# mborhi/CoMA-UNet

Measured on AMD Instinct MI355X. Metric: volumes/sec (train fwd+bwd) at 128^3 bf16, higher is better.
Workload: dtype bf16; 1 GPU; CoMA-UNet train step (fwd + RoiMSE/RnC loss + bwd + all-reduce + AdamW), 128^3 volumes, batch 2/GPU, 6-dim covariates (BASELINE configs[3]); global_batch=2, parallelism=dp1, launch=hipGraph replay of the whole step

## Files before the change

### coma_unet_amd/csrc/conv_mfma.hip

```cpp
#include "conv_mfma.h"
#include <type_traits>

template <typename T> struct elem;
template <> struct elem<bf16_t> { static constexpr int EPB = 8; };
template <> struct elem<float> { static constexpr int EPB = 4; };

__device__ __forceinline__ f32x16_t mma_piece(const uint4& a, const uint4& b, f32x16_t acc, bf16_t) {
  return __builtin_amdgcn_mfma_f32_32x32x16_bf16(*reinterpret_cast<const bf16x8_t*>(&a), *reinterpret_cast<const bf16x8_t*>(&b), acc, 0, 0, 0);
}
__device__ __forceinline__ f32x16_t mma_piece(const uint4& a, const uint4& b, f32x16_t acc, float) {
  acc = __builtin_amdgcn_mfma_f32_32x32x2f32(__uint_as_float(a.x), __uint_as_float(b.x), acc, 0, 0, 0);
  acc = __builtin_amdgcn_mfma_f32_32x32x2f32(__uint_as_float(a.y), __uint_as_float(b.y), acc, 0, 0, 0);
  acc = __builtin_amdgcn_mfma_f32_32x32x2f32(__uint_as_float(a.z), __uint_as_float(b.z), acc, 0, 0, 0);
  acc = __builtin_amdgcn_mfma_f32_32x32x2f32(__uint_as_float(a.w), __uint_as_float(b.w), acc, 0, 0, 0);
  return acc;
}

struct GatherP {
  const void* x; int ldx; long sbx; int Di, Hi, Wi, C;
  void* y; int ldy; long sby; int Do, Ho, Wo, N;
  const void* w; long wsb;
  const float* bias; int bsb;
  int k, stride, flip;
  int Mz, My, Mx;
// ... 2731 lines not shown
  extern __shared__ __attribute__((aligned(16))) char smem[];
  float* Hl = reinterpret_cast<float*>(smem);
  float* Dl = Hl + HV * CP;
  const int tid = threadIdx.x, lane = tid & 63;
  const int wid = __builtin_amdgcn_readfirstlane(tid >> 6);
  const int b = blockIdx.z;
  const int lv = lane & 15, lg = lane >> 4;
  const float* xb = p.x + (long)b * p.sbx;
  const float* db = p.dy + (long)b * p.sbn;
  const __amdgpu_buffer_rsrc_t rs_x = __builtin_amdgcn_make_buffer_rsrc(const_cast<float*>(xb), 0, p.xbytes, 0x00020000);
  const __amdgpu_buffer_rsrc_t rs_d = __builtin_amdgcn_make_buffer_rsrc(const_cast<float*>(db), 0, p.dbytes, 0x00020000);
  constexpr unsigned OOB = 0x7fff0000u;

  int s_z[NIT], s_y[NIT], s_x[NIT];
  unsigned s_boff[NIT];
#pragma unroll
  for (int it = 0; it < NIT; ++it) {
    if (it < HIT) {
      const int piece = tid + 256 * it;
      const int row = piece / PCH, ch = piece % PCH;
      const int hx = row % HX, hy = (row / HX) % HY, hz = row / (HX * HY);
      s_z[it] = piece < HP ? hz - 1 : (1 << 20); s_y[it] = hy - 1; s_x[it] = hx - 1;
      s_boff[it] = (unsigned)(ch * 16);
    } else {
      const int piece = tid + 256 * (it - HIT);
      const int row = piece / DCH, ch = piece % DCH;
      s_z[it] = row >> 7; s_y[it] = (row >> 5) & 3; s_x[it] = row & 31;
      s_boff[it] = (unsigned)(ch * 16);
    }
  }
  const int xval = p.C - 4 * (tid % PCH), dval = p.N - 4 * (tid % DCH);
  const uint4 xmask = make_uint4(xval > 0 ? ~0u : 0u, xval > 1 ? ~0u : 0u, xval > 2 ? ~0u : 0u, xval > 3 ? ~0u : 0u);
  const uint4 dmask = make_uint4(dval > 0 ? ~0u : 0u, dval > 1 ? ~0u : 0u, dval > 2 ? ~0u : 0u, dval > 3 ? ~0u : 0u);
  uint4 sreg[NIT];
  auto issue = [&](int it, int z0, int y0, int x0, const __amdgpu_buffer_rsrc_t& rx, const __amdgpu_buffer_rsrc_t& rd) __attribute__((always_inline)) {
    const int gz = z0 + s_z[it], gy = y0 + s_y[it], gx = x0 + s_x[it];
    const bool ok = (unsigned)gz < (unsigned)p.D && (unsigned)gy < (unsigned)p.H && (unsigned)gx < (unsigned)p.W;
    const int ld = it < HIT ? p.ldx : p.ldn;
    const unsigned off = (unsigned)(((gz * p.H + gy) * p.W + gx) * ld) * 4u + s_boff[it];
    const auto v = __builtin_amdgcn_raw_buffer_load_b128(it < HIT ? rx : rd, ok ? off : OOB, 0, 0);
    sreg[it] = make_uint4(v[0], v[1], v[2], v[3]);
  };
  auto store_tile = [&]() __attribute__((always_inline)) {
#pragma unroll
    for (int it = 0; it < NIT; ++it) {
      uint4 v = sreg[it];
      if (it < HIT) {
        if (tid + 256 * it < HP) {
          v.x &= xmask.x; v.y &= xmask.y; v.z &= xmask.z; v.w &= xmask.w;
          reinterpret_cast<uint4*>(Hl)[tid + 256 * it] = v;
        }
      } else {
        v.x &= dmask.x; v.y &= dmask.y; v.z &= dmask.z; v.w &= dmask.w;
        reinterpret_cast<uint4*>(Dl)[tid + 256 * (it - HIT)] = v;
      }
    }
  };

  const int gz = wid >> 1, gy0 = 2 * (wid & 1);
  const int dbase = ((gz * 4 + gy0) * 32 + lg) * ND + lv;
  const int sub = lv / CP, cc = lv % CP;
  const int xbase = ((gz * HY + gy0) * HX + lg) * CP + cc;
  int toff[NM];
#pragma unroll
  for (int m = 0; m < NM; ++m) {
    const int t = TPM == 1 ? m : (m * TPM + sub < 27 ? m * TPM + sub : 0);
    toff[m] = (((t / 9) * HY + (t / 3) % 3) * HX + t % 3) * CP;
  }
  f32x4_t acc[NM][NB];
#pragma unroll
  for (int m = 0; m < NM; ++m)
#pragma unroll
    for (int nb = 0; nb < NB; ++nb) acc[m][nb] = (f32x4_t){0.f, 0.f, 0.f, 0.f};

  const int id_begin = xcd_remap(blockIdx.x, gridDim.x) * p.ids_per_block;
  int id_end = id_begin + p.ids_per_block;
  if (id_end > p.ids_total) id_end = p.ids_total;
  int id = id_begin, tix = 0, tiy = 0, tiz = 0;
  while (id < id_end && !tile_coords(id, p.ntx, p.nty, p.ntz, tix, tiy, tiz)) ++id;
  if (id < id_end) {
#pragma unroll
    for (int it = 0; it < NIT; ++it) issue(it, tiz * TZ, tiy * TY, tix * TX, rs_x, rs_d);
  }
  while (id < id_end) {
    int nid = id + 1, ntix = 0, ntiy = 0, ntiz = 0;
    while (nid < id_end && !tile_coords(nid, p.ntx, p.nty, p.ntz, ntix, ntiy, ntiz)) ++nid;
    const bool has_next = nid < id_end;
    const __amdgpu_buffer_rsrc_t rn_x = __builtin_amdgcn_make_buffer_rsrc(const_cast<float*>(xb), 0, has_next ? p.xbytes : 0, 0x00020000);
    const __amdgpu_buffer_rsrc_t rn_d = __builtin_amdgcn_make_buffer_rsrc(const_cast<float*>(db), 0, has_next ? p.dbytes : 0, 0x00020000);
    __syncthreads();
    store_tile();
    __syncthreads();
    float af[2][NB], bf[2][NM];
    auto rd = [&](int s_, int buf) __attribute__((always_inline)) {
      const int so_d = ((s_ >> 3) * 32 + 4 * (s_ & 7)) * ND, so_x = ((s_ >> 3) * HX + 4 * (s_ & 7)) * CP;
#pragma unroll
      for (int nb = 0; nb < NB; ++nb) af[buf][nb] = Dl[dbase + so_d + nb * 16];
#pragma unroll
      for (int m = 0; m < NM; ++m) bf[buf][m] = Hl[xbase + so_x + toff[m]];
    };
    rd(0, 0);
#pragma unroll
    for (int s_ = 0; s_ < 16; ++s_) {
      if (s_ + 1 < 16) rd(s_ + 1, (s_ + 1) & 1);
      if (s_ < NIT) issue(s_, ntiz * TZ, ntiy * TY, ntix * TX, rn_x, rn_d);
      if (s_ + 16 < NIT) issue(s_ + 16, ntiz * TZ, ntiy * TY, ntix * TX, rn_x, rn_d);
      __builtin_amdgcn_sched_barrier(0);
#pragma unroll
      for (int m = 0; m < NM; ++m)
#pragma unroll
        for (int nb = 0; nb < NB; ++nb)
          acc[m][nb] = __builtin_amdgcn_mfma_f32_16x16x4f32(af[s_ & 1][nb], bf[s_ & 1][m], acc[m][nb], 0, 0, 0);
      __builtin_amdgcn_sched_barrier(0);
    }
    id = nid; tix = ntix; tiy = ntiy; tiz = ntiz;
  }
  __syncthreads();
  float* red = reinterpret_cast<float*>(smem);
  for (int i = tid; i < NM * NB * 256; i += 256) red[i] = 0.f;
  __syncthreads();
#pragma unroll
  for (int m = 0; m < NM; ++m)
#pragma unroll
    for (int nb = 0; nb < NB; ++nb)
#pragma unroll
      for (int j = 0; j < 4; ++j) atomicAdd(&red[((m * NB + nb) * 16 + 4 * lg + j) * 16 + lv], acc[m][nb][j]);
  __syncthreads();
  float* wout = p.dwk + (long)b * p.wsb + (long)(blockIdx.x % (unsigned)p.nrep) * p.rep_stride;
  for (int i = tid; i < NM * NB * 256; i += 256) {
    const int col = i & 15, row = (i >> 4) & 15, nb = (i >> 8) % NB, m = i / (256 * NB);
    const int tap = m * TPM + col / CP, c = col % CP, n = nb * 16 + row;
    if (tap < 27 && n < p.N && c < p.C) atomicAdd(wout + ((long)tap * p.N + n) * p.C + c, red[i]);
  }
}

struct Thin16WP {
  const bf16_t* x; int ldx; long sbx; int D, H, W, C;
  const bf16_t* dy; int ldn; long sbn; int N;
  unsigned xbytes, dbytes;
  int ntx, nty, ntz, ids_total, ids_per_block;
  float* dwk; long wsb;
  int nrep; long rep_stride;
};

template <int CP, int NB>
__global__ __launch_bounds__(256, 2) void conv_thin16_wgrad_k(Thin16WP p) {
  constexpr int TX = 32, TY = 4, TZ = 2, HX = TX + 2, HY = TY + 2, HZ = TZ + 2, HV = HX * HY * HZ, TM = TX * TY * TZ;
  constexpr int TPM = 16 / CP, NM = (27 + TPM - 1) / TPM;
  constexpr int ND = NB * 16;
  constexpr int PX = CP * 2, PD = ND * 2;
  constexpr int PCH = CP / 8, DCH = ND / 8;
  constexpr int HP = HV * PCH, DP = TM * DCH, HIT = (HP + 255) / 256, DIT = DP / 256, NIT = HIT + DIT;
  constexpr int RING = 8;
  extern __shared__ __attribute__((aligned(16))) char smem[];
  char* Hl = smem;
  char* Dl = smem + (HV + 2) * PX;
  const int tid = threadIdx.x, lane = tid & 63;
  const int wid = __builtin_amdgcn_readfirstlane(tid >> 6);
  const int b = blockIdx.z;
  const int lv = lane & 15, lg = lane >> 4;
  const bf16_t* xb = p.x + (long)b * p.sbx;
  const bf16_t* db = p.dy + (long)b * p.sbn;
  const __amdgpu_buffer_rsrc_t rs_x = __builtin_amdgcn_make_buffer_rsrc(const_cast<bf16_t*>(xb), 0, p.xbytes, 0x00020000);
  const __amdgpu_buffer_rsrc_t rs_d = __builtin_amdgcn_make_buffer_rsrc(const_cast<bf16_t*>(db), 0, p.dbytes, 0x00020000);
  constexpr unsigned OOB = 0x7fff0000u;

  int s_z[NIT], s_y[NIT], s_x[NIT];
#pragma unroll
  for (int it = 0; it < NIT; ++it) {
    if (it < HIT) {
      const int piece = tid + 256 * it;
      const int row = piece / PCH;
      const int hx = row % HX, hy = (row / HX) % HY, hz = row / (HX * HY);
      s_z[it] = piece < HP ? hz - 1 : (1 << 20); s_y[it] = hy - 1; s_x[it] = hx - 1;
    } else {
      const int row = (tid + 256 * (it - HIT)) / DCH;
      s_z[it] = row >> 7; s_y[it] = (row >> 5) & 3; s_x[it] = row & 31;
    }
  }
  const unsigned xoffb = (unsigned)((tid % PCH) * 16), doffb = (unsigned)((tid % DCH) * 16);
  const uint4 xmask = mask8(p.C - 8 * (tid % PCH)), dmask = mask8(p.N - 8 * (tid % DCH));
  uint4 sreg[NIT];
  auto issue = [&](int it, int z0, int y0, int x0, const __amdgpu_buffer_rsrc_t& rx, const __amdgpu_buffer_rsrc_t& rd) __attribute__((always_inline)) {
    const int gz = z0 + s_z[it], gy = y0 + s_y[it], gx = x0 + s_x[it];
    const bool ok = (unsigned)gz < (unsigned)p.D && (unsigned)gy < (unsigned)p.H && (unsigned)gx < (unsigned)p.W;
    const unsigned off = (unsigned)(((gz * p.H + gy) * p.W + gx) * (it < HIT ? p.ldx : p.ldn)) * 2u + (it < HIT ? xoffb : doffb);
    const auto v = __builtin_amdgcn_raw_buffer_load_b128(it < HIT ? rx : rd, ok ? off : OOB, 0, 0);
    sreg[it] = make_uint4(v[0], v[1], v[2], v[3]);
  };
  auto store_tile = [&]() __attribute__((always_inline)) {
#pragma unroll
    for (int it = 0; it < NIT; ++it) {
      uint4 v = sreg[it];
      if (it < HIT) {
        if (tid + 256 * it < HP) {
          v.x &= xmask.x; v.y &= xmask.y; v.z &= xmask.z; v.w &= xmask.w;
          reinterpret_cast<uint4*>(Hl)[tid + 256 * it] = v;
        }
      } else {
        v.x &= dmask.x; v.y &= dmask.y; v.z &= dmask.z; v.w &= dmask.w;
        reinterpret_cast<uint4*>(Dl)[tid + 256 * (it - HIT)] = v;
      }
    }
  };

  const int gz = wid >> 1, gy0 = 2 * (wid & 1);
  const int q4 = lv >> 2, p4 = lv & 3;
  const int vx = 4 * lg + q4;
  const int d_addr = ((gz * 4 + gy0) * 32 + vx) * PD + 8 * p4;
  const int sub = (4 * p4) / CP, cin = (4 * p4) % CP;
  const int x_addr = ((gz * HY + gy0) * HX + vx) * PX + cin * 2;
  int toff[NM];
#pragma unroll
  for (int m = 0; m < NM; ++m) {
    const int t = TPM == 1 ? m : (m * TPM + sub < 27 ? m * TPM + sub : 0);
    toff[m] = (((t / 9) * HY + (t / 3) % 3) * HX + t % 3) * PX;
  }
  f32x4_t acc[NM][NB];
#pragma unroll
  for (int m = 0; m < NM; ++m)
#pragma unroll
    for (int nb = 0; nb < NB; ++nb) acc[m][nb] = (f32x4_t){0.f, 0.f, 0.f, 0.f};

  const int id_begin = xcd_remap(blockIdx.x, gridDim.x) * p.ids_per_block;
  int id_end = id_begin + p.ids_per_block;
  if (id_end > p.ids_total) id_end = p.ids_total;
  int id = id_begin, tix = 0, tiy = 0, tiz = 0;
  while (id < id_end && !tile_coords(id, p.ntx, p.nty, p.ntz, tix, tiy, tiz)) ++id;
  if (id < id_end) {
#pragma unroll
    for (int it = 0; it < NIT; ++it) issue(it, tiz * TZ, tiy * TY, tix * TX, rs_x, rs_d);
  }
  while (id < id_end) {
    int nid = id + 1, ntix = 0, ntiy = 0, ntiz = 0;
    while (nid < id_end && !tile_coords(nid, p.ntx, p.nty, p.ntz, ntix, ntiy, ntiz)) ++nid;
    const bool has_next = nid < id_end;
    const __amdgpu_buffer_rsrc_t rn_x = __builtin_amdgcn_make_buffer_rsrc(const_cast<bf16_t*>(xb), 0, has_next ? p.xbytes : 0, 0x00020000);
    const __amdgpu_buffer_rsrc_t rn_d = __builtin_amdgcn_make_buffer_rsrc(const_cast<bf16_t*>(db), 0, has_next ? p.dbytes : 0, 0x00020000);
    __syncthreads();
    store_tile();
    __syncthreads();
    constexpr int NPAIR = 2 * NM;
    bf16x8_t bring[RING];
    auto rdb = [&](int pi) __attribute__((always_inline)) -> bf16x8_t {
      const int s_ = pi / NM, m = pi % NM;
      const char* src = Hl + x_addr + s_ * HX * PX + toff[m];
      const s4_t lo = __builtin_amdgcn_ds_read_tr16_b64_v4i16((lds_s4_t*)(src));
      const s4_t hi = __builtin_amdgcn_ds_read_tr16_b64_v4i16((lds_s4_t*)(src + 16 * PX));
      return (bf16x8_t){lo[0], lo[1], lo[2], lo[3], hi[0], hi[1], hi[2], hi[3]};
    };
    auto rda = [&](int s_, int nb) __attribute__((always_inline)) -> bf16x8_t {
      const char* src = Dl + d_addr + s_ * 32 * PD + nb * 32;
      const s4_t lo = __builtin_amdgcn_ds_read_tr16_b64_v4i16((lds_s4_t*)(src));
      const s4_t hi = __builtin_amdgcn_ds_read_tr16_b64_v4i16((lds_s4_t*)(src + 16 * PD));
      return (bf16x8_t){lo[0], lo[1], lo[2], lo[3], hi[0], hi[1], hi[2], hi[3]};
    };
    bf16x8_t afr[2][NB];
#pragma unroll
    for (int s_ = 0; s_ < 2; ++s_)
#pragma unroll
      for (int nb = 0; nb < NB; ++nb) afr[s_][nb] = rda(s_, nb);
#pragma unroll
    for (int pi = 0; pi < RING && pi < NPAIR; ++pi) bring[pi] = rdb(pi);
#pragma unroll
    for (int pi = 0; pi < NPAIR; ++pi) {
      const int s_ = pi / NM, m = pi % NM;
      const bf16x8_t bcur = bring[pi % RING];
      if (pi + RING < NPAIR) bring[pi % RING] = rdb(pi + RING);
      if (pi < NIT) issue(pi, ntiz * TZ, ntiy * TY, ntix * TX, rn_x, rn_d);
      __builtin_amdgcn_sched_barrier(0);
#pragma unroll
      for (int nb = 0; nb < NB; ++nb)
        acc[m][nb] = __builtin_amdgcn_mfma_f32_16x16x32_bf16(afr[s_][nb], bcur, acc[m][nb], 0, 0, 0);
      __builtin_amdgcn_sched_barrier(0);
    }
    static_assert(NIT <= NPAIR, "one staging piece per MFMA step");
    id = nid; tix = ntix; tiy = ntiy; tiz = ntiz;
  }
  __syncthreads();
  float* red = reinterpret_cast<float*>(smem);
  for (int i = tid; i < NM * NB * 256; i += 256) red[i] = 0.f;
  __syncthreads();
#pragma unroll
  for (int m = 0; m < NM; ++m)
#pragma unroll
    for (int nb = 0; nb < NB; ++nb)
#pragma unroll
      for (int j = 0; j < 4; ++j) atomicAdd(&red[((m * NB + nb) * 16 + 4 * lg + j) * 16 + lv], acc[m][nb][j]);
  __syncthreads();
  float* wout = p.dwk + (long)b * p.wsb + (long)(blockIdx.x % (unsigned)p.nrep) * p.rep_stride;
  for (int i = tid; i < NM * NB * 256; i += 256) {
    const int col = i & 15, row = (i >> 4) & 15, nb = (i >> 8) % NB, m = i / (256 * NB);
    const int tap = m * TPM + col / CP, c = col % CP, n = nb * 16 + row;
    if (tap < 27 && n < p.N && c < p.C) atomicAdd(wout + ((long)tap * p.N + n) * p.C + c, red[i]);
  }
}

static bool thin16_wgrad_ok(const coma_conv_desc* d, const coma_tensor* x, const coma_tensor* dy) {
  static const bool on = []{ const char* e = getenv("COMA_THIN16W"); return !(e && e[0] == '0'); }();
  const int nmax = x->C <= 8 ? 32 : 16;
  return on && d->form == 0 && d->ksize == 3 && d->stride == 1 && x->dtype == COMA_BF16 && dy->dtype == COMA_BF16 && x->W >= 32 &&
         x->C <= 16 && dy->C <= nmax && x->ld % 8 == 0 && x->sb % 8 == 0 && dy->ld % 8 == 0 && dy->sb % 8 == 0 &&
         (!x->data || aligned16(x->data)) && (!dy->data || aligned16(dy->data)) &&
         (unsigned long long)t_vox(x) * x->ld * 2 < 0x7fff0000ull && (unsigned long long)t_vox(dy) * dy->ld * 2 < 0x7fff0000ull;
}

static int conv_thin16_wgrad(const coma_conv_desc* d, const coma_tensor* x, const coma_tensor* dy, float* dwk, void* ws,
                             size_t ws_bytes, hipStream_t s, int zeroed) {
  Thin16WP q;
  q.x = (const bf16_t*)x->data; q.ldx = (int)x->ld; q.sbx = x->sb; q.D = x->D; q.H = x->H; q.W = x->W; q.C = x->C;
  q.dy = (const bf16_t*)dy->data; q.ldn = (int)dy->ld; q.sbn = dy->sb; q.N = dy->C;
  q.xbytes = (unsigned)((unsigned long long)t_vox(x) * x->ld * 2);
  q.dbytes = (unsigned)((unsigned long long)t_vox(dy) * dy->ld * 2);
  const TileRun r = tile_run(q.D, q.H, q.W, 32, 4, 2, 512, x->B);
  q.ntx = r.ntx; q.nty = r.nty; q.ntz = r.ntz; q.ids_total = r.ids_total; q.ids_per_block = r.ids_per_block;
  const long wsz1 = 27L * q.N * q.C, wsz = wsz1 * (d->per_sample_w ? x->B : 1);
  q.wsb = d->per_sample_w ? wsz1 : 0;
  const bool replicas = wsz <= WGRAD_REP_MAX_ELEMS && ws && ws_bytes >= sizeof(float) * wsz * WGRAD_NREP;
  q.nrep = replicas ? WGRAD_NREP : 1;
  q.rep_stride = replicas ? wsz : 0;
  q.dwk = replicas ? (float*)ws : dwk;
  if (!(zeroed & (replicas ? COMA_ZEROED_WS : COMA_ZEROED_OUT)) && hipMemsetAsync(q.dwk, 0, sizeof(float) * wsz * q.nrep, s) != hipSuccess) { coma_set_error("wgrad memset failed"); return 2; }
  const int cp = q.C > 8 ? 16 : 8, nb = q.N > 16 ? 2 : 1;
  const int nm = cp == 16 ? 27 : 14;
  size_t lds = (size_t)(34 * 6 * 4 + 2) * cp * 2 + (size_t)256 * nb * 16 * 2;
  if (lds < (size_t)nm * nb * 256 * 4) lds = (size_t)nm * nb * 256 * 4;
  const dim3 grid((unsigned)r.gx, 1, (unsigned)x->B);
  coma_set_kernel_tag("conv_thin16_wgrad_k<%d, %d>", cp, nb);
  if (cp == 16) hipLaunchKernelGGL((conv_thin16_wgrad_k<16, 1>), grid, dim3(256), lds, s, q);
  else if (nb == 2) hipLaunchKernelGGL((conv_thin16_wgrad_k<8, 2>), grid, dim3(256), lds, s, q);
  else hipLaunchKernelGGL((conv_thin16_wgrad_k<8, 1>), grid, dim3(256), lds, s, q);
  COMA_LAUNCH_CHECK();
  return replicas ? wgrad_replica_sum((const float*)ws, wsz, dwk, s) : 0;
}

struct F32W16P {
  const float* dn; int ldd; long sbd; int Mz, My, Mx;
  const float* ga; int ldg; long sbg; int Gz, Gy, Gx;
  int N, C;
  unsigned dbytes, gbytes;
  int ntx, nty, ntz, ids_total, ids_per_block, cblocks;
  float* dwk; long wsb;
};

template <int S, int FORM>
__global__ __launch_bounds__(256, 1) void conv_f32_wgrad16_k(F32W16P p) {
  constexpr int TX = 32, TY = S == 1 ? 4 : 2, TZ = S == 1 ? 2 : 1, TM = TX * TY * TZ;
  constexpr int HX = (TX - 1) * S + 3, HY = (TY - 1) * S + 3, HZ = (TZ - 1) * S + 3, HV = HX * HY * HZ;
  constexpr int CB = 32;
  constexpr int HIT = (HV * 8 + 255) / 256, DIT = TM * 8 / 256, NIT = HIT + DIT;
  extern __shared__ __attribute__((aligned(16))) char smem[];
  float* Hl = reinterpret_cast<float*>(smem);
  float* Dl = Hl + HV * CB;
  const int tid = threadIdx.x, lane = tid & 63;
  const int wid = __builtin_amdgcn_readfirstlane(tid >> 6);
  const int b = blockIdx.z;
  const int n0 = (blockIdx.y / p.cblocks) * CB, c0 = (blockIdx.y % p.cblocks) * CB;
  const int lv = lane & 15, lg = lane >> 4;
  const float* dnb = p.dn + (long)b * p.sbd + (FORM == 0 ? n0 : c0);
  const float* gab = p.ga + (long)b * p.sbg + (FORM == 0 ? c0 : n0);
  const __amdgpu_buffer_rsrc_t rs_g = __builtin_amdgcn_make_buffer_rsrc(const_cast<float*>(gab), 0, p.gbytes, 0x00020000);
  const __amdgpu_buffer_rsrc_t rs_d = __builtin_amdgcn_make_buffer_rsrc(const_cast<float*>(dnb), 0, p.dbytes, 0x00020000);
  constexpr unsigned OOB = 0x7fff0000u;

  const unsigned choff = (unsigned)((tid & 7) * 16);
  int s_pos[NIT];
#pragma unroll
  for (int it = 0; it < NIT; ++it) {
    if (it < HIT) {
      const int row = (tid + 256 * it) >> 3;
      const int hx = row % HX, hy = (row / HX) % HY, hz = row / (HX * HY);
      s_pos[it] = row < HV ? (hz | (hy << 4) | (hx << 8)) : (15 | (15 << 4) | (1023 << 8));
    } else {
      const int row = (tid + 256 * (it - HIT)) >> 3;
      s_pos[it] = ((row / (TY * 32)) + 1) | ((((row >> 5) % TY) + 1) << 4) | (((row & 31) + 1) << 8);
    }
  }
  uint4 sreg[NIT];
  auto issue_all = [&](int z0, int y0, int x0, const __amdgpu_buffer_rsrc_t& rg, const __amdgpu_buffer_rsrc_t& rd) __attribute__((always_inline)) {
#pragma unroll
    for (int it = 0; it < NIT; ++it) {
      const int sc = it < HIT ? S : 1;
      const int gz = sc * z0 - 1 + (s_pos[it] & 15), gy = sc * y0 - 1 + ((s_pos[it] >> 4) & 15), gx = sc * x0 - 1 + (s_pos[it] >> 8);
      const bool ok = it < HIT ? ((unsigned)gz < (unsigned)p.Gz && (unsigned)gy < (unsigned)p.Gy && (unsigned)gx < (unsigned)p.Gx)
                               : ((unsigned)gz < (unsigned)p.Mz && (unsigned)gy < (unsigned)p.My && (unsigned)gx < (unsigned)p.Mx);
      const unsigned off = it < HIT ? (unsigned)(((gz * p.Gy + gy) * p.Gx + gx) * p.ldg) * 4u + choff
                                    : (unsigned)(((gz * p.My + gy) * p.Mx + gx) * p.ldd) * 4u + choff;
      const auto v = __builtin_amdgcn_raw_buffer_load_b128(it < HIT ? rg : rd, ok ? off : OOB, 0, 0);
      sreg[it] = make_uint4(v[0], v[1], v[2], v[3]);
    }
  };
  auto store_tile = [&]() __attribute__((always_inline)) {
#pragma unroll
    for (int it = 0; it < NIT; ++it) {
      if (it < HIT) { if (((tid + 256 * it) >> 3) < HV) reinterpret_cast<uint4*>(Hl)[tid + 256 * it] = sreg[it]; }
      else reinterpret_cast<uint4*>(Dl)[tid + 256 * (it - HIT)] = sreg[it];
    }
  };

  const int nh = wid & 1, ch = wid >> 1;
  const int dbase = lg * CB + 16 * (FORM == 0 ? nh : ch) + lv;
  const int gbase = S * lg * CB + 16 * (FORM == 0 ? ch : nh) + lv;
  f32x4_t acc[27];
#pragma unroll
  for (int t = 0; t < 27; ++t) acc[t] = (f32x4_t){0.f, 0.f, 0.f, 0.f};

  const int id_begin = xcd_remap(blockIdx.x, gridDim.x) * p.ids_per_block;
  int id_end = id_begin + p.ids_per_block;
  if (id_end > p.ids_total) id_end = p.ids_total;
  int id = id_begin, tix = 0, tiy = 0, tiz = 0;
  while (id < id_end && !tile_coords(id, p.ntx, p.nty, p.ntz, tix, tiy, tiz)) ++id;
  if (id < id_end) issue_all(tiz * TZ, tiy * TY, tix * TX, rs_g, rs_d);
  while (id < id_end) {
    int nid = id + 1, ntix = 0, ntiy = 0, ntiz = 0;
    while (nid < id_end && !tile_coords(nid, p.ntx, p.nty, p.ntz, ntix, ntiy, ntiz)) ++nid;
    const bool has_next = nid < id_end;
    const __amdgpu_buffer_rsrc_t rn_g = __builtin_amdgcn_make_buffer_rsrc(const_cast<float*>(gab), 0, has_next ? p.gbytes : 0, 0x00020000);
    const __amdgpu_buffer_rsrc_t rn_d = __builtin_amdgcn_make_buffer_rsrc(const_cast<float*>(dnb), 0, has_next ? p.dbytes : 0, 0x00020000);
    __syncthreads();
    store_tile();
    __syncthreads();
    issue_all(ntiz * TZ, ntiy * TY, ntix * TX, rn_g, rn_d);
#pragma unroll 1
    for (int r = 0; r < TZ * TY; ++r) {
      const int drow = r * 32 * CB, grow = ((((r / TY) * S) * HY + (r % TY) * S) * HX) * CB;
      float df[2], gf[2][27];
      auto rd = [&](int s_, int buf) __attribute__((always_inline)) {
        df[buf] = Dl[dbase + drow + 4 * s_ * CB];
#pragma unroll
        for (int t = 0; t < 27; ++t) gf[buf][t] = Hl[gbase + grow + S * 4 * s_ * CB + (((t / 9) * HY + (t / 3) % 3) * HX + t % 3) * CB];
      };
      rd(0, 0);
#pragma unroll
      for (int s_ = 0; s_ < 8; ++s_) {
        if (s_ + 1 < 8) rd(s_ + 1, (s_ + 1) & 1);
        __builtin_amdgcn_sched_barrier(0);
#pragma unroll
        for (int t = 0; t < 27; ++t)
          acc[t] = FORM == 0 ? __builtin_amdgcn_mfma_f32_16x16x4f32(df[s_ & 1], gf[s_ & 1][t], acc[t], 0, 0, 0)
                             : __builtin_amdgcn_mfma_f32_16x16x4f32(gf[s_ & 1][t], df[s_ & 1], acc[t], 0, 0, 0);
        __builtin_amdgcn_sched_barrier(0);
      }
    }
    id = nid; tix = ntix; tiy = ntiy; tiz = ntiz;
  }
  float* wout = p.dwk + (long)b * p.wsb;
#pragma unroll
  for (int t = 0; t < 27; ++t)
#pragma unroll
    for (int j = 0; j < 4; ++j) {
      const int n = n0 + 16 * nh + 4 * lg + j, c = c0 + 16 * ch + lv;
      atomicAdd(wout + ((long)t * p.N + n) * p.C + c, acc[t][j]);
    }
}

static bool f32_wgrad16_ok(const coma_conv_desc* d, const coma_tensor* x, const coma_tensor* dy) {
  static const bool on = []{ const char* e = getenv("COMA_F32W16"); return !(e && e[0] == '0'); }();
  const coma_tensor* dn = d->form == 0 ? dy : x;
  const bool shape = d->ksize == 3 && ((d->form == 0 && (d->stride == 1 || d->stride == 2)) || (d->form == 1 && d->stride == 2));
  return on && shape && x->dtype == COMA_F32 && dy->dtype == COMA_F32 && dn->W >= 32 &&
         x->C % 32 == 0 && dy->C % 32 == 0 && x->ld % 4 == 0 && x->sb % 4 == 0 && dy->ld % 4 == 0 && dy->sb % 4 == 0 &&
         (!x->data || aligned16(x->data)) && (!dy->data || aligned16(dy->data)) &&
         (unsigned long long)t_vox(x) * x->ld * 4 < 0x7fff0000ull && (unsigned long long)t_vox(dy) * dy->ld * 4 < 0x7fff0000ull;
}

static int conv_f32_wgrad16(const coma_conv_desc* d, const coma_tensor* x, const coma_tensor* dy, float* dwk, hipStream_t s, int zeroed) {
  const coma_tensor* dn = d->form == 0 ? dy : x;
  const coma_tensor* ga = d->form == 0 ? x : dy;
  F32W16P q;
  q.dn = (const float*)dn->data; q.ldd = (int)dn->ld; q.sbd = dn->sb; q.Mz = dn->D; q.My = dn->H; q.Mx = dn->W;
  q.ga = (const float*)ga->data; q.ldg = (int)ga->ld; q.sbg = ga->sb; q.Gz = ga->D; q.Gy = ga->H; q.Gx = ga->W;
  q.N = dy->C; q.C = x->C;
  q.dbytes = (unsigned)((unsigned long long)t_vox(dn) * dn->ld * 4);
  q.gbytes = (unsigned)((unsigned long long)t_vox(ga) * ga->ld * 4);
  const int S = d->stride, tz = S == 1 ? 2 : 1, ty = S == 1 ? 4 : 2;
  q.cblocks = q.C / 32;
  const int pairs = q.cblocks * (q.N / 32);
  const TileRun r = tile_run(q.Mz, q.My, q.Mx, 32, ty, tz, 256, pairs * x->B);
  q.ntx = r.ntx; q.nty = r.nty; q.ntz = r.ntz; q.ids_total = r.ids_total; q.ids_per_block = r.ids_per_block;
  const long wsz1 = 27L * q.N * q.C, wsz = wsz1 * (d->per_sample_w ? x->B : 1);
  q.wsb = d->per_sample_w ? wsz1 : 0;
  q.dwk = dwk;
  if (!(zeroed & COMA_ZEROED_OUT) && hipMemsetAsync(dwk, 0, sizeof(float) * wsz, s) != hipSuccess) { coma_set_error("wgrad memset failed"); return 2; }
  const size_t lds = S == 1 ? (size_t)(34 * 6 * 4 + 256) * 32 * 4 : (size_t)(65 * 5 * 3 + 64) * 32 * 4;
// ... 312 lines not shown
```

Before: 117.7 volumes/s.

## Double-buffer LDS in thin16 wgrad kernel to overlap staging with MFMA

The thin-channel weight-gradient kernel now keeps two LDS images. The next tile's register-staged loads are stored into the spare image during the current tile's MFMA loop, and loads for the tile after that are issued in the same loop. This removes the per-tile store-and-barrier bubble in favour of a single barrier per tile, and keeps global loads two tiles ahead. In exchange LDS use roughly doubles (with a raised max-LDS attribute), which may lower occupancy from the requested 2 blocks per CU. An A/B profiling script is also added.

Measured after the change: 117.5 volumes/s. Within noise of the previous version (-0.1%).

```diff
diff --git a/coma_unet_amd/csrc/conv_mfma.hip b/coma_unet_amd/csrc/conv_mfma.hip
--- a/coma_unet_amd/csrc/conv_mfma.hip
+++ b/coma_unet_amd/csrc/conv_mfma.hip
@@ -2907,17 +2907,15 @@
   constexpr int PCH = CP / 8, DCH = ND / 8;
   constexpr int HP = HV * PCH, DP = TM * DCH, HIT = (HP + 255) / 256, DIT = DP / 256, NIT = HIT + DIT;
   constexpr int RING = 8;
+  constexpr int HBY = HIT * 256 * 16, IMG = HBY + TM * PD;
+  static_assert(HBY >= (HV + 2) * PX, "the padding taps' reads stay inside the halo part");
   extern __shared__ __attribute__((aligned(16))) char smem[];
-  char* Hl = smem;
-  char* Dl = smem + (HV + 2) * PX;
   const int tid = threadIdx.x, lane = tid & 63;
   const int wid = __builtin_amdgcn_readfirstlane(tid >> 6);
   const int b = blockIdx.z;
   const int lv = lane & 15, lg = lane >> 4;
   const bf16_t* xb = p.x + (long)b * p.sbx;
   const bf16_t* db = p.dy + (long)b * p.sbn;
-  const __amdgpu_buffer_rsrc_t rs_x = __builtin_amdgcn_make_buffer_rsrc(const_cast<bf16_t*>(xb), 0, p.xbytes, 0x00020000);
-  const __amdgpu_buffer_rsrc_t rs_d = __builtin_amdgcn_make_buffer_rsrc(const_cast<bf16_t*>(db), 0, p.dbytes, 0x00020000);
   constexpr unsigned OOB = 0x7fff0000u;
 
   int s_z[NIT], s_y[NIT], s_x[NIT];
@@ -2934,35 +2932,29 @@
     }
   }
   const unsigned xoffb = (unsigned)((tid % PCH) * 16), doffb = (unsigned)((tid % DCH) * 16);
-  const uint4 xmask = mask8(p.C - 8 * (tid % PCH)), dmask = mask8(p.N - 8 * (tid % DCH));
-  uint4 sreg[NIT];
+  typedef unsigned tw_u32x4_t __attribute__((ext_vector_type(4)));
+  const uint4 xm_ = mask8(p.C - 8 * (tid % PCH)), dm_ = mask8(p.N - 8 * (tid % DCH));
+  const tw_u32x4_t xmask = {xm_.x, xm_.y, xm_.z, xm_.w}, dmask = {dm_.x, dm_.y, dm_.z, dm_.w};
+  tw_u32x4_t sreg[NIT];
+  auto rsrc = [&](const bf16_t* base, unsigned bytes, bool live) __attribute__((always_inline)) {
+    return __builtin_amdgcn_make_buffer_rsrc(const_cast<bf16_t*>(base), 0, live ? bytes : 0, 0x00020000);
+  };
   auto issue = [&](int it, int z0, int y0, int x0, const __amdgpu_buffer_rsrc_t& rx, const __amdgpu_buffer_rsrc_t& rd) __attribute__((always_inline)) {
     const int gz = z0 + s_z[it], gy = y0 + s_y[it], gx = x0 + s_x[it];
     const bool ok = (unsigned)gz < (unsigned)p.D && (unsigned)gy < (unsigned)p.H && (unsigned)gx < (unsigned)p.W;
     const unsigned off = (unsigned)(((gz * p.H + gy) * p.W + gx) * (it < HIT ? p.ldx : p.ldn)) * 2u + (it < HIT ? xoffb : doffb);
-    const auto v = __builtin_amdgcn_raw_buffer_load_b128(it < HIT ? rx : rd, ok ? off : OOB, 0, 0);
-    sreg[it] = make_uint4(v[0], v[1], v[2], v[3]);
-  };
-  auto store_tile = [&]() __attribute__((always_inline)) {
-#pragma unroll
-    for (int it = 0; it < NIT; ++it) {
-      uint4 v = sreg[it];
-      if (it < HIT) {
-        if (tid + 256 * it < HP) {
-          v.x &= xmask.x; v.y &= xmask.y; v.z &= xmask.z; v.w &= xmask.w;
-          reinterpret_cast<uint4*>(Hl)[tid + 256 * it] = v;
-        }
-      } else {
-        v.x &= dmask.x; v.y &= dmask.y; v.z &= dmask.z; v.w &= dmask.w;
-        reinterpret_cast<uint4*>(Dl)[tid + 256 * (it - HIT)] = v;
-      }
-    }
-  };
+    sreg[it] = __builtin_amdgcn_raw_buffer_load_b128(it < HIT ? rx : rd, ok ? off : OOB, 0, 0);
+  };
+  const int st_addr = tid * 16;
+  auto store_piece = [&](int it, int img) __attribute__((always_inline)) {
+    *reinterpret_cast<tw_u32x4_t*>(smem + img + st_addr + 4096 * it) = sreg[it] & (it < HIT ? xmask : dmask);
+  };
+  static_assert(HBY == HIT * 4096, "dy pieces follow the halo pieces at the same 4096-byte step");
 
   const int gz = wid >> 1, gy0 = 2 * (wid & 1);
   const int q4 = lv >> 2, p4 = lv & 3;
   const int vx = 4 * lg + q4;
-  const int d_addr = ((gz * 4 + gy0) * 32 + vx) * PD + 8 * p4;
+  const int d_addr = HBY + ((gz * 4 + gy0) * 32 + vx) * PD + 8 * p4;
   const int sub = (4 * p4) / CP, cin = (4 * p4) % CP;
   const int x_addr = ((gz * HY + gy0) * HX + vx) * PX + cin * 2;
   int toff[NM];
@@ -2982,30 +2974,39 @@
   if (id_end > p.ids_total) id_end = p.ids_total;
   int id = id_begin, tix = 0, tiy = 0, tiz = 0;
   while (id < id_end && !tile_coords(id, p.ntx, p.nty, p.ntz, tix, tiy, tiz)) ++id;
-  if (id < id_end) {
-#pragma unroll
-    for (int it = 0; it < NIT; ++it) issue(it, tiz * TZ, tiy * TY, tix * TX, rs_x, rs_d);
-  }
+  int nid = id + 1, ntix = 0, ntiy = 0, ntiz = 0;
+  while (nid < id_end && !tile_coords(nid, p.ntx, p.nty, p.ntz, ntix, ntiy, ntiz)) ++nid;
+  {
+    const __amdgpu_buffer_rsrc_t r0_x = rsrc(xb, p.xbytes, id < id_end), r0_d = rsrc(db, p.dbytes, id < id_end);
+    const __amdgpu_buffer_rsrc_t r1_x = rsrc(xb, p.xbytes, nid < id_end), r1_d = rsrc(db, p.dbytes, nid < id_end);
+#pragma unroll
+    for (int it = 0; it < NIT; ++it) issue(it, tiz * TZ, tiy * TY, tix * TX, r0_x, r0_d);
+#pragma unroll
+    for (int it = 0; it < NIT; ++it) {
+      store_piece(it, 0);
+      issue(it, ntiz * TZ, ntiy * TY, ntix * TX, r1_x, r1_d);
+    }
+  }
+  __syncthreads();
+  int cur = 0;
   while (id < id_end) {
-    int nid = id + 1, ntix = 0, ntiy = 0, ntiz = 0;
-    while (nid < id_end && !tile_coords(nid, p.ntx, p.nty, p.ntz, ntix, ntiy, ntiz)) ++nid;
-    const bool has_next = nid < id_end;
-    const __amdgpu_buffer_rsrc_t rn_x = __builtin_amdgcn_make_buffer_rsrc(const_cast<bf16_t*>(xb), 0, has_next ? p.xbytes : 0, 0x00020000);
-    const __amdgpu_buffer_rsrc_t rn_d = __builtin_amdgcn_make_buffer_rsrc(const_cast<bf16_t*>(db), 0, has_next ? p.dbytes : 0, 0x00020000);
-    __syncthreads();
-    store_tile();
-    __syncthreads();
+    int nnid = nid + 1, nntix = 0, nntiy = 0, nntiz = 0;
+    while (nnid < id_end && !tile_coords(nnid, p.ntx, p.nty, p.ntz, nntix, nntiy, nntiz)) ++nnid;
+    const __amdgpu_buffer_rsrc_t rn_x = rsrc(xb, p.xbytes, nnid < id_end), rn_d = rsrc(db, p.dbytes, nnid < id_end);
+    const int oth = cur ^ IMG;
+    const char* Hl = smem + cur + x_addr;
+    const char* Dl = smem + cur + d_addr;
     constexpr int NPAIR = 2 * NM;
     bf16x8_t bring[RING];
     auto rdb = [&](int pi) __attribute__((always_inline)) -> bf16x8_t {
       const int s_ = pi / NM, m = pi % NM;
-      const char* src = Hl + x_addr + s_ * HX * PX + toff[m];
+      const char* src = Hl + s_ * HX * PX + toff[m];
       const s4_t lo = __builtin_amdgcn_ds_read_tr16_b64_v4i16((lds_s4_t*)(src));
       const s4_t hi = __builtin_amdgcn_ds_read_tr16_b64_v4i16((lds_s4_t*)(src + 16 * PX));
       return (bf16x8_t){lo[0], lo[1], lo[2], lo[3], hi[0], hi[1], hi[2], hi[3]};
     };
     auto rda = [&](int s_, int nb) __attribute__((always_inline)) -> bf16x8_t {
-      const char* src = Dl + d_addr + s_ * 32 * PD + nb * 32;
+      const char* src = Dl + s_ * 32 * PD + nb * 32;
       const s4_t lo = __builtin_amdgcn_ds_read_tr16_b64_v4i16((lds_s4_t*)(src));
       const s4_t hi = __builtin_amdgcn_ds_read_tr16_b64_v4i16((lds_s4_t*)(src + 16 * PD));
       return (bf16x8_t){lo[0], lo[1], lo[2], lo[3], hi[0], hi[1], hi[2], hi[3]};
@@ -3022,7 +3023,10 @@
       const int s_ = pi / NM, m = pi % NM;
       const bf16x8_t bcur = bring[pi % RING];
       if (pi + RING < NPAIR) bring[pi % RING] = rdb(pi + RING);
-      if (pi < NIT) issue(pi, ntiz * TZ, ntiy * TY, ntix * TX, rn_x, rn_d);
+      if (pi < NIT) {
+        store_piece(pi, oth);
+        issue(pi, nntiz * TZ, nntiy * TY, nntix * TX, rn_x, rn_d);
+      }
       __builtin_amdgcn_sched_barrier(0);
 #pragma unroll
       for (int nb = 0; nb < NB; ++nb)
@@ -3030,10 +3034,13 @@
       __builtin_amdgcn_sched_barrier(0);
     }
     static_assert(NIT <= NPAIR, "one staging piece per MFMA step");
+    __syncthreads();
     id = nid; tix = ntix; tiy = ntiy; tiz = ntiz;
-  }
-  __syncthreads();
+    nid = nnid; ntix = nntix; ntiy = nntiy; ntiz = nntiz;
+    cur = oth;
+  }
   float* red = reinterpret_cast<float*>(smem);
+  static_assert(NM * NB * 256 * 4 <= 2 * IMG, "red fits in the two images");
   for (int i = tid; i < NM * NB * 256; i += 256) red[i] = 0.f;
   __syncthreads();
 #pragma unroll
@@ -3077,14 +3084,15 @@
   q.dwk = replicas ? (float*)ws : dwk;
   if (!(zeroed & (replicas ? COMA_ZEROED_WS : COMA_ZEROED_OUT)) && hipMemsetAsync(q.dwk, 0, sizeof(float) * wsz * q.nrep, s) != hipSuccess) { coma_set_error("wgrad memset failed"); return 2; }
   const int cp = q.C > 8 ? 16 : 8, nb = q.N > 16 ? 2 : 1;
-  const int nm = cp == 16 ? 27 : 14;
-  size_t lds = (size_t)(34 * 6 * 4 + 2) * cp * 2 + (size_t)256 * nb * 16 * 2;
-  if (lds < (size_t)nm * nb * 256 * 4) lds = (size_t)nm * nb * 256 * 4;
+  const size_t hit = ((size_t)34 * 6 * 4 * (cp / 8) + 255) / 256;
+  const size_t lds = 2 * (hit * 4096 + (size_t)256 * nb * 16 * 2);
   const dim3 grid((unsigned)r.gx, 1, (unsigned)x->B);
   coma_set_kernel_tag("conv_thin16_wgrad_k<%d, %d>", cp, nb);
-  if (cp == 16) hipLaunchKernelGGL((conv_thin16_wgrad_k<16, 1>), grid, dim3(256), lds, s, q);
-  else if (nb == 2) hipLaunchKernelGGL((conv_thin16_wgrad_k<8, 2>), grid, dim3(256), lds, s, q);
-  else hipLaunchKernelGGL((conv_thin16_wgrad_k<8, 1>), grid, dim3(256), lds, s, q);
+#define THIN16W(CP_, NB_) do { set_max_lds<conv_thin16_wgrad_k<CP_, NB_>, 80>(); hipLaunchKernelGGL((conv_thin16_wgrad_k<CP_, NB_>), grid, dim3(256), lds, s, q); } while (0)
+  if (cp == 16) THIN16W(16, 1);
+  else if (nb == 2) THIN16W(8, 2);
+  else THIN16W(8, 1);
+#undef THIN16W
   COMA_LAUNCH_CHECK();
   return replicas ? wgrad_replica_sum((const float*)ws, wsz, dwk, s) : 0;
 }
diff --git a/profiles/thin_wgrad_ab.py b/profiles/thin_wgrad_ab.py
--- /dev/null
+++ b/profiles/thin_wgrad_ab.py
@@ -0,0 +1,168 @@
+import argparse
+import json
+import os
+import statistics
+import subprocess
+import sys
+
+ROOT = os.path.dirname(os.path.dirname(os.path.abspath(__file__)))
+SHAPES = [(1, 32, True, 8, 32), (16, 1, False, 16, 8), (16, 16, False, 16, 16), (2, 8, False, 8, 8), (3, 16, False, 8, 16),
+          (8, 1, False, 8, 8), (8, 8, False, 8, 8)]
+SIZE, BATCH, ITERS, ROUNDS, RUNS = 128, 2, 20, 5, 5
+
+
+def _name(sh):
+    return f"{sh[0]}->{sh[1]}{' per-sample' if sh[2] else ''}"
+
+
+def _mbytes(sh):
+    up8 = lambda n: (n + 7) // 8 * 8
+    return BATCH * SIZE ** 3 * 2 * (up8(sh[0]) + up8(sh[1])) / 1e6
+
+
+def launch():
+    import torch
+    sys.path.insert(0, ROOT)
+    from coma_unet_amd import ops, _lib as L
+    out = {}
+    for sh in SHAPES:
+        C, N, ps, ldx, ldn = sh
+        g = torch.Generator(device="cuda").manual_seed(1)
+        x = torch.randn((BATCH, SIZE, SIZE, SIZE, ldx), generator=g, device="cuda").bfloat16()[..., :C]
+        dy = torch.randn((BATCH, SIZE, SIZE, SIZE, ldn), generator=g, device="cuda").bfloat16()[..., :N]
+        d = ops._desc(3, 1, 0, ps, 0)
+        cx, cdy = L.ct(x), L.ct(dy)
+        nws = L.lib.coma_conv_wgrad_ws_bytes(d, cx, cdy)
+        ws = torch.zeros((nws,), dtype=torch.uint8, device="cuda")
+        dw = torch.zeros((BATCH if ps else 1, 27, N, C), device="cuda")
+        ev = [(torch.cuda.Event(enable_timing=True), torch.cuda.Event(enable_timing=True)) for _ in range(ITERS)]
+        for it in range(-3, ITERS):
+            if it >= 0:
+                ev[it][0].record()
+            L.check(L.lib.coma_conv_wgrad(d, cx, cdy, L.ptr(dw), None, L.ptr(ws), nws, L.ZEROED_OUT | L.ZEROED_WS, L.stream()), "wgrad")
+            if it >= 0:
+                ev[it][1].record()
+        torch.cuda.synchronize()
+        tag = L.lib.coma_last_kernel().decode()
+        assert tag.startswith("conv_thin16_wgrad_k"), tag
+        out[_name(sh)] = [statistics.median(a.elapsed_time(b) * 1e3 for a, b in ev), tag]
+        del x, dy, ws, dw
+    print("RESULT " + json.dumps(out))
+
+
+def _child(cmd, cwd, env, limit):
+    p = subprocess.run(cmd, cwd=cwd, env=env, timeout=limit, stdout=subprocess.PIPE, stderr=subprocess.PIPE, text=True)
+    if p.returncode != 0:
+        sys.stdout.write(p.stdout[-2000:] + p.stderr[-4000:])
+        sys.exit(f"child failed with status {p.returncode}: {' '.join(cmd)}; nothing further is started")
+    print(f"done: {' '.join(cmd[1:])} in {cwd}", file=sys.stderr, flush=True)
+    return p.stdout
+
+
+def _stats(v):
+    return statistics.median(v), min(v), max(v)
+
+
+def ab_launch(parent):
+    arms = {"parent": os.path.join(parent, "coma_unet_amd", "libcoma_unet.so"), "this": os.path.join(ROOT, "coma_unet_amd", "libcoma_unet.so")}
+    got = {a: {_name(s): [] for s in SHAPES} for a in arms}
+    tags = {}
+    for r in range(ROUNDS):
+        for arm, lib in arms.items():
+            out = _child([sys.executable, os.path.abspath(__file__), "launch"], ROOT, dict(os.environ, COMA_UNET_LIB=lib), 180)
+            res = json.loads([ln for ln in out.splitlines() if ln.startswith("RESULT ")][-1][7:])
+            for k, (us, tag) in res.items():
+                got[arm][k].append(us)
+                tags[k] = tag
+    print(f"# per launch, us: median [min .. max] of {ROUNDS} processes per arm (each the median of {ITERS} launches), 128^3, batch 2, bf16")
+    print(f"{'layer':>18s} {'kernel':>28s} {'MB':>5s}  {'parent':>24s} {'this tree':>24s}  {'TB/s':>11s}  verdict")
+    ok = True
+    for sh in SHAPES:
+        k = _name(sh)
+        (mp, lp, hp), (mt, lt, ht) = _stats(got["parent"][k]), _stats(got["this"][k])
+        met = mp - mt > max(hp - lp, ht - lt)
+        ok &= met
+        mb = _mbytes(sh)
+        print(f"{k:>18s} {tags[k]:>28s} {mb:5.0f}  {mp:7.1f} [{lp:6.1f} .. {hp:6.1f}] {mt:7.1f} [{lt:6.1f} .. {ht:6.1f}]  "
+              f"{mb / mp:4.2f} -> {mb / mt:4.2f}  {'MET' if met else 'NOT MET'} ({mp / mt:.2f}x)")
+    print("ALL ROWS MET" if ok else "SOME ROWS NOT MET")
+
+
+def _bench(tree, extra, limit=300):
+    out = _child([sys.executable, "bench.py", "--gpus", "1"] + extra, tree, dict(os.environ), limit)
+    return json.loads([ln for ln in out.splitlines() if ln.startswith("{")][-1])
+
+
+def ab_step(parent):
+    got = {"parent": [], "this": []}
+    for r in range(RUNS):
+        for arm, tree in (("parent", parent), ("this", ROOT)):
+            got[arm].append(float(_bench(tree, ["--steps", "20", "--warmup", "5"])["ms_per_step"]))
+    print("# python bench.py --gpus 1 --steps 20 --warmup 5 (128^3, batch 2, bf16, graph replay), alternating; ms per step")
+    for arm, label in (("parent", "parent commit"), ("this", "this tree")):
+        m, lo, hi = _stats(got[arm])
+        print(f"{label:14s} " + " ".join(f"{v:.3f}" for v in got[arm]) + f"   median {m:.3f}  min {lo:.3f}  max {hi:.3f}  spread {hi - lo:.3f}")
+    if max(got["this"]) < min(got["parent"]):
+        print(f"The sets do not overlap: the slowest run of this tree ({max(got['this']):.3f}) is faster than the fastest of the parent ({min(got['parent']):.3f}).")
+    else:
+        print("The sets OVERLAP: no claim on the step time from this run.")
+
+
+def dumps(parent, out):
+    import numpy as np
+    dirs = {}
+    for tag, tree in (("parent1", parent), ("parent2", parent), ("this1", ROOT)):
+        dirs[tag] = os.path.join(os.path.abspath(out), tag)
+        _bench(tree, ["--steps", "5", "--warmup", "2", "--dump-outputs", dirs[tag]])
+    rel = lambda a, b: float(np.linalg.norm(a.astype(np.float64) - b) / max(np.linalg.norm(b.astype(np.float64)), 1e-300))
+    print("# bench.py --dump-outputs of parent run 1, parent run 2 and this tree: rel-L2 per array against parent run 1; rule this/parent <= 4 x parent/parent")
+    print(f"{'array':>22s} {'parent/parent':>14s} {'this/parent':>14s}  4x rule")
+    bad = False
+    for f in sorted(os.listdir(dirs["parent1"])):
+        a, b, c = (np.load(os.path.join(dirs[t], f)) for t in ("parent1", "parent2", "this1"))
+        pp, tp = rel(b, a), rel(c, a)
+        okay = tp <= 4 * pp
+        bad |= not okay
+        print(f"{f[:-4]:>22s} {pp:14.3e} {tp:14.3e}  {'ok' if okay else 'ABOVE'}")
+    print("SOME ARRAYS ABOVE 4x" if bad else "ALL ARRAYS WITHIN 4x")
+
+
+def populations(parent, out, n=3):
+    import itertools
+    import numpy as np
+    dirs = {"parent": [], "this": []}
+    for i in range(n):
+        for arm, tree in (("parent", parent), ("this", ROOT)):
+            dirs[arm].append(os.path.join(os.path.abspath(out), f"{arm}{i}"))
+            _bench(tree, ["--steps", "5", "--warmup", "2", "--dump-outputs", dirs[arm][-1]])
+    rel = lambda a, b: float(np.linalg.norm(a.astype(np.float64) - b) / max(np.linalg.norm(b.astype(np.float64)), 1e-300))
+    print(f"# {n} dumps per tree (bench.py --steps 5 --warmup 2 --dump-outputs, alternating), every pair, rel-L2 sorted")
+    for f in sorted(os.listdir(dirs["parent"][0])):
+        ld = {arm: [np.load(os.path.join(d, f)) for d in dirs[arm]] for arm in dirs}
+        rows = {"parent/parent": [rel(a, b) for a, b in itertools.combinations(ld["parent"], 2)],
+                "this/this": [rel(a, b) for a, b in itertools.combinations(ld["this"], 2)],
+                "this/parent": [rel(a, b) for a in ld["this"] for b in ld["parent"]]}
+        if max(max(v) for v in rows.values()) == 0.0:
+            continue
+        for k, v in rows.items():
+            print(f"{f[:-4]:>18s} {k:>14s}: " + " ".join(f"{x:.2e}" for x in sorted(v)))
+
+
+if __name__ == "__main__":
+    ap = argparse.ArgumentParser()
+    ap.add_argument("what", choices=["launch", "ab-launch", "ab-step", "dumps", "populations"])
+    ap.add_argument("--parent")
+    ap.add_argument("--out", default=None)
+    a = ap.parse_args()
+    if a.what == "launch":
+        launch()
+    elif a.what == "ab-launch":
+        ab_launch(os.path.abspath(a.parent))
+    elif a.what == "ab-step":
+        ab_step(os.path.abspath(a.parent))
+    elif a.what == "populations":
+        import tempfile
+        populations(os.path.abspath(a.parent), a.out or tempfile.mkdtemp())
+    else:
+        import tempfile
+        dumps(os.path.abspath(a.parent), a.out or tempfile.mkdtemp())
```
